# life-ufes/multimodal-model-skin-lesion-classifier

Hardware: AMD Instinct MI355X
Metric: images/sec fwd+bwd, ResNet-50+crossattention bs=256 (higher is better)
Workload: dtype bf16; 1 GPU; ResNet-50 + one-hot(20) + crossattention, 224x224, train step incl. Adam; per_gpu_batch=256, global_batch=256, parallelism=dp1, weights=random init (torchvision / timm / transformers layouts), unfreeze_weights=unfrozen_weights, linear_dtype=fp32

## Files before the change

### include/mmskin.h

```cpp
#ifndef MMSKIN_H
#define MMSKIN_H
#include <stdint.h>

#ifdef __cplusplus
extern "C" {
#endif

#define MMSKIN_F32 0
#define MMSKIN_BF16 1

const char* mmskin_last_error(void);
int mmskin_version(void);

typedef struct mmskin_backbone* mmskin_backbone_t;
int mmskin_backbone_create(const char* arch, int batch, int height, int width, int dtype, mmskin_backbone_t* out);
void mmskin_backbone_destroy(mmskin_backbone_t h);
int mmskin_backbone_num_tensors(mmskin_backbone_t h, int kind );
int mmskin_backbone_tensor_info(mmskin_backbone_t h, int kind, int index, char* name, int name_cap,
                                int64_t* offset, int64_t* numel, int* ndim, int64_t* shape4);
int64_t mmskin_backbone_param_numel(mmskin_backbone_t h);
int64_t mmskin_backbone_buffer_numel(mmskin_backbone_t h);
int64_t mmskin_backbone_workspace_bytes(mmskin_backbone_t h);
int mmskin_backbone_feature_dim(mmskin_backbone_t h);
int mmskin_backbone_feature_hw(mmskin_backbone_t h, int* out_h, int* out_w);
// ... 112 lines not shown
                                  void* stream);
int64_t mmskin_adaptive_avgpool_workspace_bytes(int N, int C, int H, int W);
int mmskin_adaptive_avgpool_forward(const float* x, float* out, int N, int C, int H, int W, int dtype, void* workspace, void* stream);
int mmskin_adaptive_avgpool_backward(const float* dout, float* dx, int N, int C, int H, int W, int dtype, void* workspace, void* stream);
int64_t mmskin_stem_workspace_bytes(int N, int H, int W);
int mmskin_stem_forward(const float* x, const float* w, const float* gamma, const float* beta, float* y, int N, int H,
                        int W, float eps, int dtype, void* workspace, void* stream);
int mmskin_stem_backward(const float* dy, const float* x, const float* w, const float* gamma, const float* beta,
                         float* dw, float* dgamma, float* dbeta, int N, int H, int W, float eps, int dtype,
                         void* workspace, void* stream);

int mmskin_linear_forward(const float* x, const float* w, const float* b, float* y, int M, int K, int N, int relu,
                          void* stream);
int mmskin_linear_backward(const float* dy, const float* x, const float* w, const float* y_relu, float* dy_scratch,
                           float* dx, float* dw, float* db, int M, int K, int N, void* stream);
int mmskin_linear_gelu_backward(const float* dh, const float* x, const float* w, const float* z, float* dy_scratch, float* dx, float* dw,
                                float* db, int M, int K, int N, void* stream);
int mmskin_linear_x16_pitch(int M, int K, int N);
enum { MMSKIN_LINEAR_SMALL = 0, MMSKIN_LINEAR_BIG_F32 = 1, MMSKIN_LINEAR_BIG_BF16 = 2, MMSKIN_LINEAR_PADDED_BF16 = 3 };
int mmskin_linear_route(int M, int K, int N);
int mmskin_linear_forward_keep(const float* x, const float* w, const float* b, const float* res, float* y, void* x16_keep, int M, int K,
                               int N, int relu, void* stream);
int mmskin_linear_backward_keep(const float* dy, const void* x16, const float* w, const float* y_relu, const float* z_gelu, float* dy_scratch,
                                float* dx, float* dw, float* db, int M, int K, int N, void* stream);
int mmskin_gelu_forward_bf16(const float* z, void* h16, int64_t rows, int cols, int cols_pad, void* stream);
int mmskin_linear_forward_x16(const void* x16, const float* w, const float* b, const float* res, float* y, int M, int K, int N, int relu,
                              void* stream);
int mmskin_star_relu_forward_bf16(const float* z, const float* s, const float* b, void* h16, int64_t rows, int cols, int cols_pad,
                                  void* stream);
int mmskin_linear_star_relu_backward_keep(const float* dh, const void* x16, const float* w, const float* z, const float* s, float* dsb,
// ... 201 lines not shown
```

### multimodal-model-skin-lesion-classifier_amd/csrc/linear.hip

```cpp
#include <stdlib.h>
#include <string.h>

#include "../../include/mmskin.h"
#include "conv.h"
#include "head_internal.h"

float* head_scratch(size_t bytes, int slot) {
  constexpr int MAXDEV = 16;
  static float* buf[2][MAXDEV] = {};
  static size_t cap[2][MAXDEV] = {};
  int d = 0;
  if (hipGetDevice(&d) != hipSuccess || d < 0 || d >= MAXDEV) return nullptr;
  if (bytes > cap[slot][d]) {
    if (buf[slot][d]) (void)hipFree(buf[slot][d]);
    size_t want = bytes < (size_t)(8 << 20) ? (size_t)(8 << 20) : bytes;
    if (hipMalloc((void**)&buf[slot][d], want) != hipSuccess) { buf[slot][d] = nullptr; cap[slot][d] = 0; return nullptr; }
    cap[slot][d] = want;
  }
  return buf[slot][d];
}
__global__ void split_reduce_kernel(const float* __restrict__ part, float* __restrict__ out, int S, int64_t n) {
  for (int64_t i = blockIdx.x * (int64_t)blockDim.x + threadIdx.x; i < n; i += (int64_t)gridDim.x * blockDim.x) {
    float t = 0.f;
    for (int s2 = 0; s2 < S; ++s2) t += part[(int64_t)s2 * n + i];
// ... 68 lines not shown
                                                       int64_t sbk, int64_t ldc, int relu, int kchunk, int64_t sab,
                                                       int64_t sbb, int64_t scb) {
  __shared__ float As[LG_LDS];
  __shared__ float Bs[LG_LDS];
  if (kchunk < 0) {
    a += (int64_t)blockIdx.z * sab; b += (int64_t)blockIdx.z * sbb; c += (int64_t)blockIdx.z * scb;
  }
  if (kchunk > 0) {
    const int kb = blockIdx.z * kchunk;
    a += (int64_t)kb * sak; b += (int64_t)kb * sbk;
    c += (int64_t)blockIdx.z * M * ldc;
    K = min(kchunk, K - kb);
  }
  gemm_f32_tile<A_KC, B_KC>(a, b, c, bias, M, N, K, sam, sak, sbn, sbk, ldc, relu, blockIdx.x, blockIdx.y, As, Bs);
}
__global__ __launch_bounds__(256) void linear_bwd_small_kernel(const float* __restrict__ g, const float* __restrict__ w, const float* __restrict__ x,
                                                               float* __restrict__ dx, float* __restrict__ dw, float* __restrict__ db, int M, int K,
                                                               int N, int nx_dx, int n_dx, int nx_dw, int n_dw) {
  __shared__ float As[LG_LDS];
  __shared__ float Bs[LG_LDS];
  int b = blockIdx.x;
  if (b < n_dx) {
    gemm_f32_tile<true, false>(g, w, dx, nullptr, M, K, N, N, 1, 1, K, K, 0, b % nx_dx, b / nx_dx, As, Bs);
    return;
  }
  b -= n_dx;
  if (b < n_dw) {
    gemm_f32_tile<false, false>(g, x, dw, nullptr, N, K, M, 1, N, 1, K, K, 0, b % nx_dw, b / nx_dw, As, Bs);
    return;
  }
  b -= n_dw;
  const int cx = threadIdx.x & 31, ry = threadIdx.x >> 5, n = b * 32 + cx;
  float s0 = 0.f, s1 = 0.f, s2 = 0.f, s3 = 0.f;
  if (n < N) {
    int m = ry;
    for (; m + 24 < M; m += 32) {
      s0 += g[(int64_t)m * N + n]; s1 += g[(int64_t)(m + 8) * N + n]; s2 += g[(int64_t)(m + 16) * N + n]; s3 += g[(int64_t)(m + 24) * N + n];
    }
    for (; m < M; m += 8) s0 += g[(int64_t)m * N + n];
  }
  As[ry * 32 + cx] = (s0 + s1) + (s2 + s3);
  __syncthreads();
  if (ry == 0 && n < N) {
    float t = 0.f;
#pragma unroll
    for (int i = 0; i < 8; ++i) t += As[i * 32 + cx];
    db[n] = t;
  }
}

static int gemm_f32(const float* a, const float* b, float* c, const float* bias, int M, int N, int K, int64_t sam,
                    int64_t sak, int64_t sbn, int64_t sbk, int64_t ldc, int relu, hipStream_t st, int batch = 1,
                    int64_t sab = 0, int64_t sbb = 0, int64_t scb = 0) {
  if (M <= 0 || N <= 0) return MMSKIN_OK;
  dim3 grid(ceil_div(N, LG_T), ceil_div(M, LG_T));
  const bool akc = sak == 1, bkc = sbk == 1;
  int S = 1, kchunk = 0;
  float* out = c;
  const int tiles = grid.x * grid.y;
  if (batch > 1) {
    grid.z = batch;
  } else if (K >= 4096 && tiles < 256 && !bias && !relu && ldc == N) {
    S = ceil_div(512, tiles);
// ... 480 lines not shown
  }
  if (path == LIN_BIG_F32) {
    ConvShape s = {M, 1, 1, K, N, 1, 1, 1, 0};
    FwdFuse f; f.bias = b; f.relu = relu == 1; f.gelu = relu == 2;
    return launch_conv_fwd<float>(s, x, w, y, nullptr, nullptr, st, (b || relu) ? &f : nullptr);
  }
  rc = gemm_f32(x, w, y, b, M, N, K, K, 1, K, 1, N, relu == 1, st);
  if (rc || relu != 2) return rc;
  return mmskin_gelu_forward(y, y, (int64_t)M * N, stream);
}

struct LinearBwdOpt {
  const void* x16_kept = nullptr;
  const float* star_s = nullptr;
  float* star_sb = nullptr;
};
static int linear_backward_impl(const float* dy, const float* x, const float* w, const float* y_relu, const float* z_gelu, float* dy_scratch,
                                float* dx, float* dw, float* db, int M, int K, int N, void* stream, const LinearBwdOpt& o = LinearBwdOpt()) {
  ARG_CHECK(dy && M > 0 && K > 0 && N > 0, "linear_backward: bad argument");
  ARG_CHECK(!(y_relu && z_gelu), "linear_backward: one activation");
  hipStream_t st = ST(stream);
  const float* g = dy;
  const LinearPath path = linear_path(M, K, N);
  const bool bf16_gemm = linear_bf16_gemm(path);
  ARG_CHECK(!o.x16_kept || bf16_gemm, "linear_backward: the kept bf16 operand belongs to the bf16 large-GEMM path (mode changed since the forward?)");
  ARG_CHECK(!o.star_s || (bf16_gemm && z_gelu && o.star_sb), "linear_backward: StarReLU needs the bf16 large-GEMM path, z and the scalar gradients");
  int rc;
  if (z_gelu && !bf16_gemm) {
    ARG_CHECK(dy_scratch, "linear_backward: dy_scratch required with z_gelu");
    if ((rc = mmskin_gelu_backward(dy, z_gelu, dy_scratch, (int64_t)M * N, stream))) return rc;
    g = dy_scratch; z_gelu = nullptr;
  }
  if (y_relu) {
    ARG_CHECK(dy_scratch, "linear_backward: dy_scratch required with y_relu");
    hipLaunchKernelGGL(relu_mask_kernel, dim3(grid1d((int64_t)M * N)), dim3(256), 0, st, dy, y_relu, dy_scratch, (int64_t)M * N);
    HIP_CHECK_RET(hipGetLastError());
    g = dy_scratch;
  }
  if (bf16_gemm) {
    const bool padded = path == LIN_PADDED_BF16;
    const int Kp = padded ? pad64(K) : K, Np = padded ? pad64(N) : N;
    ConvShape s = {M, 1, 1, Kp, Np, 1, 1, 1, 0};
    const size_t slab_bytes = conv_wgrad_slab_bytes(s);
    const size_t star_floats = o.star_s ? (size_t)2 * colsum4_blocks(M, Np / 4) : 0;
    bf16_t *g16 = nullptr, *t16 = nullptr, *w16 = nullptr;
    WgradSlab slab = {nullptr, slab_bytes / sizeof(float)};
    float *star_part = nullptr, *part = nullptr;
    const bool placed = carve_scratch([&](Carver& c) {
      g16 = c.take<bf16_t>((size_t)M * Np);
      t16 = c.take<bf16_t>((size_t)M * Kp);
      w16 = c.take<bf16_t>((size_t)Np * Kp);
      slab.p = reinterpret_cast<float*>(c.take<unsigned char>(slab_bytes));
      if (star_floats) star_part = c.take<float>(star_floats);
// ... 40 lines not shown
    });
    if (!placed) { mmskin_set_error("linear_backward: scratch allocation failed"); return MMSKIN_ERR_HIP; }
    if (dx) {
      ARG_CHECK(w, "linear_backward: w required for dx");
      hipLaunchKernelGGL(transpose_f32_kernel, dim3(ceil_div(K, 32), ceil_div(N, 32)), dim3(32, 8), 0, st, w, wt, N, K);
      HIP_CHECK_RET(hipGetLastError());
      if ((rc = launch_conv_dgrad<float>(s, g, wt, dx, (const float*)nullptr, st))) return rc;
    }
    if (dw) {
      ARG_CHECK(x, "linear_backward: x required for dw");
      if ((rc = launch_conv_wgrad<float>(s, g, x, slab, dw, st))) return rc;
    }
    if (db && (rc = colsum(g, db, M, N, st))) return rc;
    return MMSKIN_OK;
  }
  if (M < 4096 && (dx || dw || db)) {
    ARG_CHECK((!dx || w) && (!dw || x), "linear_backward: w / x required");
    const int nx_dx = ceil_div(K, LG_T), n_dx = dx ? nx_dx * ceil_div(M, LG_T) : 0;
    const int nx_dw = ceil_div(K, LG_T), n_dw = dw ? nx_dw * ceil_div(N, LG_T) : 0;
    const int n_db = db ? ceil_div(N, 32) : 0;
    hipLaunchKernelGGL(linear_bwd_small_kernel, dim3(n_dx + n_dw + n_db), dim3(256), 0, st, g, w, x, dx, dw, db, M, K, N, nx_dx, n_dx, nx_dw, n_dw);
    HIP_CHECK_RET(hipGetLastError());
    return MMSKIN_OK;
  }
  if (dx) {
    ARG_CHECK(w, "linear_backward: w required for dx");
    if ((rc = gemm_f32(g, w, dx, nullptr, M, K, N, N, 1, 1, K, K, 0, st))) return rc;
  }
  if (dw) {
    ARG_CHECK(x, "linear_backward: x required for dw");
    if ((rc = gemm_f32(g, x, dw, nullptr, N, K, M, 1, N, 1, K, K, 0, st))) return rc;
  }
  if (db && (rc = colsum(g, db, M, N, st))) return rc;
  return MMSKIN_OK;
}

// ... 71 lines not shown
            "linear_lane: dtype / activation");
  ARG_CHECK(drop_p >= 0.f && drop_p < 1.f, "linear_lane: dropout probability %f", (double)drop_p);
  ARG_CHECK(linear_path(M, K, N) == LIN_BIG_BF16, "linear_lane: M=%d K=%d N=%d is off the large bf16 GEMM path (rows >= 2048, 64-multiple widths, "
            "MMSKIN_LINEAR_DTYPE=bf16)", M, K, N);
  const bool tr = gamma || residual || drop_p > 0.f;
  ARG_CHECK(!tr || (y_dtype == 0 && N % 128 == 0), "linear_lane: residual / layer scale / dropout need an fp32 result and N %% 128 == 0");
  FwdFuse f; f.bias = b; f.relu = act == 1; f.gelu = act == 2;
  f.gamma = gamma; f.res_f32 = residual; f.drop_p = drop_p; f.seed = seed; f.offset = offset;
  return linear_big_bf16_ex(x, x_dtype, w, w_dtype, f, b || act || tr, y, y_dtype, M, K, N, "linear_lane", ST(stream));
}

int mmskin_linear_backward(const float* dy, const float* x, const float* w, const float* y_relu, float* dy_scratch,
                           float* dx, float* dw, float* db, int M, int K, int N, void* stream) {
  return linear_backward_impl(dy, x, w, y_relu, nullptr, dy_scratch, dx, dw, db, M, K, N, stream);
}
int mmskin_linear_gelu_backward(const float* dh, const float* x, const float* w, const float* z, float* dy_scratch, float* dx, float* dw,
                                float* db, int M, int K, int N, void* stream) {
  ARG_CHECK(z, "linear_gelu_backward: z required");
  return linear_backward_impl(dh, x, w, nullptr, z, dy_scratch, dx, dw, db, M, K, N, stream);
}
int mmskin_linear_backward_keep(const float* dy, const void* x16, const float* w, const float* y_relu, const float* z_gelu, float* dy_scratch,
                                float* dx, float* dw, float* db, int M, int K, int N, void* stream) {
  ARG_CHECK(x16, "linear_backward_keep: x16 required");
  LinearBwdOpt o; o.x16_kept = x16;
  return linear_backward_impl(dy, nullptr, w, y_relu, z_gelu, dy_scratch, dx, dw, db, M, K, N, stream, o);
}

int mmskin_linear_star_relu_backward_keep(const float* dh, const void* x16, const float* w, const float* z, const float* s, float* dsb,
                                          float* dx, float* dw, float* db, int M, int K, int N, void* stream) {
  ARG_CHECK(x16 && z && s && dsb, "linear_star_relu_backward_keep: x16, z, s and dsb required");
// ... 25 lines not shown
```

### multimodal-model-skin-lesion-classifier_amd/mmskin/_lib.py

```python
import ctypes
import os
import re

_HERE = os.path.dirname(os.path.abspath(__file__))
LIB_PATH = os.path.join(os.path.dirname(_HERE), "libmmskin_hip.so")
HEADER_PATH = os.path.join(os.path.dirname(os.path.dirname(_HERE)), "include", "mmskin.h")

F32, BF16 = 0, 1
LINEAR_SMALL, LINEAR_BIG_F32, LINEAR_BIG_BF16, LINEAR_PADDED_BF16 = 0, 1, 2, 3
WG_STAGED, WG_TAPS3, WG_RING, WG_RING3 = 0, 1, 2, 3
WGR_DIRECT, WGR_LANES = 0, 1
CG_TILE128, CG_BIG256, CG_PIPE, CG_C64, CG_STEM7 = 0, 1, 2, 3, 4

_lib = None

c_f = ctypes.c_void_p
_i, _i64, _f = ctypes.c_int, ctypes.c_int64, ctypes.c_float
_u64 = ctypes.c_uint64
_P = ctypes.c_void_p

_SIGNATURES = {
    "mmskin_last_error": (ctypes.c_char_p, []),
    "mmskin_version": (_i, []),
    "mmskin_backbone_create": (_i, [ctypes.c_char_p, _i, _i, _i, _i, ctypes.POINTER(_P)]),
    "mmskin_backbone_destroy": (None, [_P]),
    "mmskin_backbone_num_tensors": (_i, [_P, _i]),
    "mmskin_backbone_tensor_info": (_i, [_P, _i, _i, ctypes.c_char_p, _i, ctypes.POINTER(_i64),
                                         ctypes.POINTER(_i64), ctypes.POINTER(_i), ctypes.POINTER(_i64)]),
    "mmskin_backbone_param_numel": (_i64, [_P]),
    "mmskin_backbone_buffer_numel": (_i64, [_P]),
    "mmskin_backbone_workspace_bytes": (_i64, [_P]),
    "mmskin_backbone_feature_dim": (_i, [_P]),
    "mmskin_backbone_feature_hw": (_i, [_P, _P, _P]),
    "mmskin_backbone_set_option": (_i, [_P, ctypes.c_char_p, _i]),
# ... 60 lines not shown
    "mmskin_slice_stats_workspace_bytes": (_i64, [_i64, _i, _i, _i]),
    "mmskin_col_reduce_scratch_doubles": (_i64, [_i64]),
    "mmskin_col_reduce_scratch_check": (_i, [_i, _i, _i, _i64]),
    "mmskin_slice_stats": (_i, [_P, _i64, _i, _i, _i, _P, _P, _i, _P, _P]),
    "mmskin_maxpool2_relu_workspace_bytes": (_i64, [_i] * 4),
    "mmskin_maxpool2_relu_forward": (_i, [_P] * 3 + [_i] * 5 + [_P, _P]),
    "mmskin_maxpool2_relu_backward": (_i, [_P] * 3 + [_i] * 5 + [_P, _P]),
    "mmskin_adaptive_avgpool_workspace_bytes": (_i64, [_i] * 4),
    "mmskin_adaptive_avgpool_forward": (_i, [_P] * 2 + [_i] * 5 + [_P, _P]),
    "mmskin_adaptive_avgpool_backward": (_i, [_P] * 2 + [_i] * 5 + [_P, _P]),
    "mmskin_stem_workspace_bytes": (_i64, [_i] * 3),
    "mmskin_stem_forward": (_i, [_P] * 5 + [_i] * 3 + [_f, _i, _P, _P]),
    "mmskin_stem_backward": (_i, [_P] * 8 + [_i] * 3 + [_f, _i, _P, _P]),
    "mmskin_linear_forward": (_i, [_P] * 4 + [_i] * 4 + [_P]),
    "mmskin_linear_backward": (_i, [_P] * 8 + [_i] * 3 + [_P]),
    "mmskin_linear_gelu_backward": (_i, [_P] * 8 + [_i] * 3 + [_P]),
    "mmskin_linear_x16_pitch": (_i, [_i, _i, _i]),
    "mmskin_linear_route": (_i, [_i, _i, _i]),
    "mmskin_linear_forward_keep": (_i, [_P] * 6 + [_i] * 4 + [_P]),
    "mmskin_linear_backward_keep": (_i, [_P] * 9 + [_i] * 3 + [_P]),
    "mmskin_gelu_forward_bf16": (_i, [_P, _P, _i64, _i, _i, _P]),
    "mmskin_linear_forward_x16": (_i, [_P] * 5 + [_i] * 4 + [_P]),
    "mmskin_layernorm_forward": (_i, [_P] * 6 + [_i, _i, _f, _i, _P]),
    "mmskin_layernorm_backward": (_i, [_P] * 9 + [_i, _i, _i, _P]),
    "mmskin_sigmoid_gate_forward": (_i, [_P] * 3 + [_i64, _P]),
    "mmskin_sigmoid_gate_backward": (_i, [_P] * 5 + [_i64, _P]),
    "mmskin_gated_mix_forward": (_i, [_P] * 4 + [_i64, _P]),
    "mmskin_gated_mix_backward": (_i, [_P] * 7 + [_i64, _P]),
    "mmskin_metablock_gate_forward": (_i, [_P] * 4 + [_i64, _P]),
    "mmskin_metablock_gate_backward": (_i, [_P] * 7 + [_i64, _P]),
# ... 138 lines not shown
```

### multimodal-model-skin-lesion-classifier_amd/mmskin/nn.py

```python
import torch
import torch.nn as nn

from . import ops


class HipLinear(nn.Linear):
    def __init__(self, in_features, out_features, bias=True, fuse_relu=False):
        super().__init__(in_features, out_features, bias=bias)
        self.fuse_relu = fuse_relu

    def forward(self, x):
        return ops.linear(x, self.weight, self.bias, self.fuse_relu)

    def extra_repr(self):
        return super().extra_repr() + (", fused_relu=True" if self.fuse_relu else "")


class HipLayerNorm(nn.LayerNorm):
    def __init__(self, normalized_shape, fuse_relu=False):
        super().__init__(normalized_shape)
        self.fuse_relu = fuse_relu

    def forward(self, x):
        return ops.layernorm(x, self.weight, self.bias, self.eps, self.fuse_relu)
# ... 45 lines not shown
            v = ops.linear_rows(value.reshape(B, D), W, Bv, 2 * D, 3 * D)
            o = ops.linear(v, self.out_proj.weight, self.out_proj.bias).reshape(1, B, D)
            if Lq != 1:
                o = o.expand(Lq, B, D)
        else:
            q = ops.linear(query.reshape(Lq * B, D), W[:D], Bv[:D] if Bv is not None else None)
            k = ops.linear(key.reshape(Lk * B, D), W[D:2 * D], Bv[D:2 * D] if Bv is not None else None)
            v = ops.linear(value.reshape(Lk * B, D), W[2 * D:], Bv[2 * D:] if Bv is not None else None)
            split = lambda t, L: t.reshape(L, B, H, D // H).permute(1, 2, 0, 3).contiguous()
            a = ops.attention(split(q, Lq), split(k, Lk), split(v, Lk), self.dropout, self.training)
            a = a.permute(2, 0, 1, 3).reshape(Lq * B, D)
            o = ops.linear(a, self.out_proj.weight, self.out_proj.bias).reshape(Lq, B, D)
        if self.batch_first:
            o = o.transpose(0, 1)
        return o, None
```

### multimodal-model-skin-lesion-classifier_amd/mmskin/ops.py

```python
import ctypes
import weakref

import numpy as np
import torch

from . import _lib
from ._autograd import (_dropout_counter, _dropout_state, _dtype_code, _f32c, _need_gpu, _needs_grad, get_linear_dtype,
                        no_second_order)
from ._lib import call, ptr, stream
from .attention import (LongAttentionFn, _bmm, attention, attention_blhd, attention_packed, attention_route,
                        channel_attention, channel_attention_ok, window_attention, window_attention_ok)


def set_linear_dtype(name):
    call("mmskin_set_linear_dtype", {"fp32": _lib.F32, "float32": _lib.F32, "bf16": _lib.BF16, "bfloat16": _lib.BF16}[name.lower()])


def _linear_forward(x, w, b, res, act, want_keep):
    x2 = _f32c(x).reshape(-1, x.shape[-1])
    w = _f32c(w)
    M, K = x2.shape
    N = w.shape[0]
    y = torch.empty((M, N), device=x.device, dtype=torch.float32)
    pitch = _lib.load().mmskin_linear_x16_pitch(M, K, N) if want_keep else 0
# ... 60 lines not shown
             M, K, N, 0, stream())
        ctx.save_for_backward(x2 if ctx.needs_input_grad[1] else None, w)
        ctx.rows, ctx.mk, ctx.xshape = (r0, r1), (M, K), x.shape
        ctx.bias = None if b is None else (b.shape, b.dtype)
        return y.reshape(*x.shape[:-1], N)

    @staticmethod
    def backward(ctx, dy):
        xs, w = ctx.saved_tensors
        (r0, r1), (M, K) = ctx.rows, ctx.mk
        N = r1 - r0
        dy2 = _f32c(dy).reshape(M, N)
        need_x, need_w = ctx.needs_input_grad[0], ctx.needs_input_grad[1]
        need_b = ctx.bias is not None and ctx.needs_input_grad[2]
        dx = torch.empty((M, K), device=dy.device, dtype=torch.float32) if need_x else None
        nw, nb = (w.numel() if need_w else 0), (ctx.bias[0].numel() if need_b else 0)
        flat = torch.zeros(nw + nb, device=dy.device, dtype=torch.float32) if nw + nb else None
        dw = flat[:nw].view_as(w) if need_w else None
        db = flat[nw:].view(ctx.bias[0]) if need_b else None
        call("mmskin_linear_backward", ptr(dy2), ptr(xs), w.data_ptr() + 4 * r0 * K, None, None, ptr(dx),
             (dw.data_ptr() + 4 * r0 * K) if need_w else None, (db.data_ptr() + 4 * r0) if need_b else None, M, K, N, stream())
        return (dx.reshape(ctx.xshape) if need_x else None), dw, db, None, None


def linear_rows(x, w, b, r0, r1):
    if x.dtype != torch.float32 or not x.is_cuda:
        return linear(x, w[r0:r1], b[r0:r1] if b is not None else None)
    return LinearRowsFn.apply(x, w, b, r0, r1)


def _rows_f32_or_bf16(x):
    x2 = x.reshape(-1, x.shape[-1]).contiguous()
    return x2 if x2.dtype in (torch.float32, torch.bfloat16) else x2.float()


def lane_dtype(x, module=None, *tensors):
    if not x.is_cuda or get_linear_dtype() != "bf16":
        return None
    params = tuple(module.parameters()) if module is not None else ()
    return None if _needs_grad(x, *params, *tensors) else torch.bfloat16


def _linear_ex(x, w, b, act, out_dtype):
# ... 944 lines not shown
```

### multimodal-model-skin-lesion-classifier_amd/models/gatedResidualBlock.py

```python
import os
import sys

import torch.nn as nn

_PKG = os.path.dirname(os.path.dirname(os.path.abspath(__file__)))
if _PKG not in sys.path:
    sys.path.insert(0, _PKG)

from mmskin import ops
from mmskin.nn import HipDropout, HipLayerNorm, HipLinear, HipMultiheadAttention


class GatedAlteredResidualBlock(nn.Module):
    def __init__(self, dim, dropout=0.1):
        super().__init__()
        self.norm = HipLayerNorm(dim)
        self.attn = HipMultiheadAttention(embed_dim=dim, num_heads=8, batch_first=False)
        self.dropout = HipDropout(dropout)
        self.gate_linear = HipLinear(dim, dim)

    def forward(self, q, k, v):
        a = self.dropout(self.attn(q, k, v)[0])
        z = self.gate_linear(q)
        return self.norm(ops.gated_mix(z, a.expand_as(q) if a.shape != q.shape else a, q))


class StackedGatedResidualBlock(nn.Module):
    def __init__(self, dim, depth=4, dropout=0.1):
        super().__init__()
        self.blocks = nn.ModuleList(
            [GatedAlteredResidualBlock(dim=dim, dropout=dropout) for _ in range(depth)])

    def forward(self, q, k=None, v=None):
        k = q if k is None else k
        v = q if v is None else v
        for block in self.blocks:
            q = block(q, k, v)
        return q
```

### multimodal-model-skin-lesion-classifier_amd/models/multimodalIntraInterModal.py

```python
import os
import sys

import torch
import torch.nn as nn

_HERE = os.path.dirname(os.path.abspath(__file__))
_PKG = os.path.dirname(_HERE)
for _p in (_PKG, _HERE):
    if _p not in sys.path:
        sys.path.insert(0, _p)

from gatedResidualBlock import GatedAlteredResidualBlock, StackedGatedResidualBlock
from loadImageModelClassifier import loadModels
from metablock import MetaBlock
from mmskin import ops
from mmskin.nn import FusedAway, HipDropout, HipLayerNorm, HipLinear, HipMultiheadAttention

_RG = "att-intramodal+residual+cross-attention-metadados"


class MultimodalModel(nn.Module):
    def __init__(self, num_classes, num_heads, device, cnn_model_name, text_model_name, batch_size=32,
                 common_dim=512, text_encoder_dim_output=512, vocab_size=91,
                 unfreeze_weights="frozen_weights", attention_mecanism="concatenation", n=2):
        super().__init__()
        self.device = device
        self.common_dim = common_dim
        self.num_heads = num_heads
        self.attention_mecanism = attention_mecanism
        self.n = n
        self.vocab_size = vocab_size
# ... 71 lines not shown
            img_feat = img_feat.mean(dim=(-2, -1))
        return img_feat

    def forward(self, image, text_metadata):
        return self.fuse(self.encode_image(image), text_metadata)

    def fuse(self, img_feat, text_metadata):
        mech = self.attention_mecanism
        needs_meta = mech not in ("no-metadata", "no-metadata-without-mlp")
        if mech == "no-metadata-without-mlp":
            return self.fc_visual_only(img_feat)
        txt_feat = self._metadata_features(text_metadata) if needs_meta else None
        if mech == "metablock":
            return self.fc_mlp_module_after_metablock_fusion_module(self.meta_block(img_feat, txt_feat))

        P_i = self.image_projector(img_feat).unsqueeze(0)
        if mech == "no-metadata":
            return self.fc_fusion(P_i.squeeze(0))
        P_t = self.text_projector(txt_feat).unsqueeze(0)

        isa, tsa = self.image_self_attention, self.text_self_attention
        ica, tca = self.image_cross_attention, self.text_cross_attention
        ires, tres = self.image_residual, self.text_residual
        att = lambda mod, q, kv: mod(q, kv, kv)[0]
        fuse = lambda a, b: self.fc_fusion(ops.concat2(a.squeeze(0), b.squeeze(0)))
        f2o = self.fc_fusion_proj_feat2output

        if mech == "concatenation":
            return fuse(P_i, P_t)
        if mech == "weighted":
            return fuse(ops.sigmoid_gate(self.img_gate(P_i), P_i), ops.sigmoid_gate(self.txt_gate(P_t), P_t))
        if mech == "rg-att2fusefeatures":
            return f2o(ires(P_t, P_i, P_i).squeeze(0))
        if mech == "rg-att":
            return fuse(ires(P_i, P_t, P_t), tres(P_t, P_i, P_i))
        if mech == "cross-attention-only":
            return fuse(att(ica, P_i, P_t), att(tca, P_t, P_i))
        if mech == "residual+cross-attention-metadados":
            R_i, R_t = ires(P_i, P_i, P_i), tres(P_t, P_t, P_t)
            return fuse(att(ica, R_i, R_t), att(tca, R_t, R_i))

        A_i, A_t = att(isa, P_i, P_i), att(tsa, P_t, P_t)
        if mech == "att-intramodal":
            return fuse(A_i, A_t)
        if mech == "att-intramodal+residual":
            return fuse(ires(P_i, A_i, A_i), tres(P_t, A_t, A_t))
        if mech in ("crossattention", "gfcam", "cross-weights-after-crossattention"):
            C_i, C_t = att(ica, A_i, A_t), att(tca, A_t, A_i)
            if mech == "crossattention":
                return fuse(C_i, C_t)
            z_i, z_t = self.img_gate(C_i), self.txt_gate(C_t)
            if mech == "gfcam":
                return fuse(ops.sigmoid_gate(z_i, C_i), ops.sigmoid_gate(z_t, C_t))
            return fuse(ops.sigmoid_gate(z_t, C_i), ops.sigmoid_gate(z_i, C_t))
        if mech.startswith(_RG):
            R_i, R_t = ires(P_i, A_i, A_i), tres(P_t, A_t, A_t)
            X_i, X_t = att(ica, R_i, R_t), att(tca, R_t, R_i)
            tail = mech[len(_RG):]
            if tail == "":
                return fuse(X_i, X_t)
            if tail == "+rg-att2fusefeatures":
                return f2o(ires(X_t, X_i, X_i).squeeze(0))
            if tail == "+metablock":
                return f2o(self.meta_block(X_i.squeeze(0), X_t.squeeze(0)))
            if tail == "+att-intramodal+residual":
                A2_i, A2_t = att(isa, X_i, X_i), att(tsa, X_t, X_t)
                return fuse(ires(X_i, A2_i, A2_i), tres(X_t, A2_t, A2_t))
        raise ValueError(f"Attention mechanism '{mech}' not implemented.")
```

Baseline: 14710 images/sec.

## Batch paired image/text head linears and attention into single paired kernel launches

Adds forward and backward paired-linear kernels that run two independent small fp32 linear problems (image and text branch) in one launch using a 2-D grid. The crossattention model's projectors, self/cross attention (sequence-length-1 shortcut through the value and out projections) and gates now go through these paired paths. Backward also folds the zeroing of unused weight-gradient rows into the same kernel instead of separate memsets. The aim is to cut kernel-launch and Python dispatch overhead in the tiny head layers, at the cost of more complex autograd plumbing and grids that idle when the two problems differ in size.

Measured after the change: 14840 images/sec (median of 6 runs). Within noise of the previous version (+0.9%).

```diff
diff --git a/include/mmskin.h b/include/mmskin.h
--- a/include/mmskin.h
+++ b/include/mmskin.h
@@ -150,6 +150,17 @@
                           void* stream);
 int mmskin_linear_backward(const float* dy, const float* x, const float* w, const float* y_relu, float* dy_scratch,
                            float* dx, float* dw, float* db, int M, int K, int N, void* stream);
+typedef struct mmskin_linear_fwd_desc {
+  const float* x; const float* w; const float* b; float* y;
+  int M, K, N, act, r0, r1;
+} mmskin_linear_fwd_desc;
+typedef struct mmskin_linear_bwd_desc {
+  const float* dy; const float* x; const float* w; const float* y_relu; float* dy_scratch; float* dx; float* dw; float* db;
+  int M, K, N, r0, r1;
+} mmskin_linear_bwd_desc;
+int mmskin_linear_forward_pair(const mmskin_linear_fwd_desc* a, const mmskin_linear_fwd_desc* b, void* stream);
+int mmskin_linear_backward_pair(const mmskin_linear_bwd_desc* a, const mmskin_linear_bwd_desc* b, void* stream);
+int64_t mmskin_linear_pair_launches(void);
 int mmskin_linear_gelu_backward(const float* dh, const float* x, const float* w, const float* z, float* dy_scratch, float* dx, float* dw,
                                 float* db, int M, int K, int N, void* stream);
 int mmskin_linear_x16_pitch(int M, int K, int N);
diff --git a/multimodal-model-skin-lesion-classifier_amd/csrc/linear.hip b/multimodal-model-skin-lesion-classifier_amd/csrc/linear.hip
--- a/multimodal-model-skin-lesion-classifier_amd/csrc/linear.hip
+++ b/multimodal-model-skin-lesion-classifier_amd/csrc/linear.hip
@@ -106,39 +106,83 @@
   }
   gemm_f32_tile<A_KC, B_KC>(a, b, c, bias, M, N, K, sam, sak, sbn, sbk, ldc, relu, blockIdx.x, blockIdx.y, As, Bs);
 }
-__global__ __launch_bounds__(256) void linear_bwd_small_kernel(const float* __restrict__ g, const float* __restrict__ w, const float* __restrict__ x,
-                                                               float* __restrict__ dx, float* __restrict__ dw, float* __restrict__ db, int M, int K,
-                                                               int N, int nx_dx, int n_dx, int nx_dw, int n_dw) {
+#define LB_ZERO 4096
+struct LinBwdProb {
+  const float *g, *w, *x;
+  float *dx, *dw, *db;
+  int M, K, N;
+  int nx_dx, n_dx, nx_dw, n_dw, n_db, n_zero;
+  int r0, nw;
+};
+static inline int lin_bwd_blocks(const LinBwdProb& p) { return p.n_dx + p.n_dw + p.n_db + p.n_zero; }
+__device__ __forceinline__ void linear_bwd_small_block(const LinBwdProb& p, int b, float* As, float* Bs) {
+  const float* __restrict__ g = p.g;
+  const int M = p.M, K = p.K, N = p.N;
+  if (b < p.n_dx) {
+    gemm_f32_tile<true, false>(g, p.w, p.dx, nullptr, M, K, N, N, 1, 1, K, K, 0, b % p.nx_dx, b / p.nx_dx, As, Bs);
+    return;
+  }
+  b -= p.n_dx;
+  if (b < p.n_dw) {
+    gemm_f32_tile<false, false>(g, p.x, p.dw, nullptr, N, K, M, 1, N, 1, K, K, 0, b % p.nx_dw, b / p.nx_dw, As, Bs);
+    return;
+  }
+  b -= p.n_dw;
+  if (b < p.n_db) {
+    const int cx = threadIdx.x & 31, ry = threadIdx.x >> 5, n = b * 32 + cx;
+    float s0 = 0.f, s1 = 0.f, s2 = 0.f, s3 = 0.f;
+    if (n < N) {
+      int m = ry;
+      for (; m + 24 < M; m += 32) {
+        s0 += g[(int64_t)m * N + n]; s1 += g[(int64_t)(m + 8) * N + n]; s2 += g[(int64_t)(m + 16) * N + n]; s3 += g[(int64_t)(m + 24) * N + n];
+      }
+      for (; m < M; m += 8) s0 += g[(int64_t)m * N + n];
+    }
+    As[ry * 32 + cx] = (s0 + s1) + (s2 + s3);
+    __syncthreads();
+    if (ry == 0 && n < N) {
+      float t = 0.f;
+#pragma unroll
+      for (int i = 0; i < 8; ++i) t += As[i * 32 + cx];
+      p.db[n] = t;
+    }
+    return;
+  }
+  b -= p.n_db;
+  const int64_t zw = p.dw ? (int64_t)(p.nw - N) * K : 0, zt = zw + (p.db ? p.nw - N : 0);
+  const int64_t lo = (int64_t)p.r0 * K;
+  float* __restrict__ dw0 = p.dw - lo;
+  float* __restrict__ db0 = p.db - p.r0;
+  const int64_t end = min((int64_t)(b + 1) * LB_ZERO, zt);
+  for (int64_t i = (int64_t)b * LB_ZERO + threadIdx.x; i < end; i += 256) {
+    if (i < zw) dw0[i < lo ? i : i + (int64_t)N * K] = 0.f;
+    else { const int64_t j = i - zw; db0[j < p.r0 ? j : j + N] = 0.f; }
+  }
+}
+__global__ __launch_bounds__(256) void linear_bwd_small_kernel(LinBwdProb p) {
   __shared__ float As[LG_LDS];
   __shared__ float Bs[LG_LDS];
-  int b = blockIdx.x;
-  if (b < n_dx) {
-    gemm_f32_tile<true, false>(g, w, dx, nullptr, M, K, N, N, 1, 1, K, K, 0, b % nx_dx, b / nx_dx, As, Bs);
-    return;
-  }
-  b -= n_dx;
-  if (b < n_dw) {
-    gemm_f32_tile<false, false>(g, x, dw, nullptr, N, K, M, 1, N, 1, K, K, 0, b % nx_dw, b / nx_dw, As, Bs);
-    return;
-  }
-  b -= n_dw;
-  const int cx = threadIdx.x & 31, ry = threadIdx.x >> 5, n = b * 32 + cx;
-  float s0 = 0.f, s1 = 0.f, s2 = 0.f, s3 = 0.f;
-  if (n < N) {
-    int m = ry;
-    for (; m + 24 < M; m += 32) {
-      s0 += g[(int64_t)m * N + n]; s1 += g[(int64_t)(m + 8) * N + n]; s2 += g[(int64_t)(m + 16) * N + n]; s3 += g[(int64_t)(m + 24) * N + n];
-    }
-    for (; m < M; m += 8) s0 += g[(int64_t)m * N + n];
-  }
-  As[ry * 32 + cx] = (s0 + s1) + (s2 + s3);
-  __syncthreads();
-  if (ry == 0 && n < N) {
-    float t = 0.f;
-#pragma unroll
-    for (int i = 0; i < 8; ++i) t += As[i * 32 + cx];
-    db[n] = t;
-  }
+  linear_bwd_small_block(p, blockIdx.x, As, Bs);
+}
+struct LinFwdProb {
+  const float *x, *w, *b;
+  float* y;
+  int M, K, N, relu, nx, nblk;
+};
+__global__ __launch_bounds__(256) void linear_fwd_pair_kernel(LinFwdProb p0, LinFwdProb p1) {
+  __shared__ float As[LG_LDS];
+  __shared__ float Bs[LG_LDS];
+  const LinFwdProb& p = blockIdx.y ? p1 : p0;
+  const int b = blockIdx.x;
+  if (b >= p.nblk) return;
+  gemm_f32_tile<true, true>(p.x, p.w, p.y, p.b, p.M, p.N, p.K, p.K, 1, p.K, 1, p.N, p.relu, b % p.nx, b / p.nx, As, Bs);
+}
+__global__ __launch_bounds__(256) void linear_bwd_pair_kernel(LinBwdProb p0, LinBwdProb p1) {
+  __shared__ float As[LG_LDS];
+  __shared__ float Bs[LG_LDS];
+  const LinBwdProb& p = blockIdx.y ? p1 : p0;
+  if ((int)blockIdx.x >= p.n_dx + p.n_dw + p.n_db + p.n_zero) return;
+  linear_bwd_small_block(p, blockIdx.x, As, Bs);
 }
 
 static int gemm_f32(const float* a, const float* b, float* c, const float* bias, int M, int N, int K, int64_t sam,
@@ -649,7 +693,34 @@
   const void* x16_kept = nullptr;
   const float* star_s = nullptr;
   float* star_sb = nullptr;
+  int r0 = 0, nw = 0;
 };
+static inline bool linear_bwd_one_launch(LinearPath path, int M) { return path == LIN_SMALL && M < 4096; }
+static inline bool linear_fwd_one_launch(LinearPath path, int K, int act) { return path == LIN_SMALL && K < 4096 && act != 2; }
+static LinBwdProb lin_bwd_prob(const float* g, const float* w, const float* x, float* dx, float* dw, float* db, int M, int K, int N, int r0,
+                               int nw) {
+  LinBwdProb p = {g, w, x, dx, dw, db, M, K, N};
+  p.nx_dx = ceil_div(K, LG_T); p.n_dx = dx ? p.nx_dx * ceil_div(M, LG_T) : 0;
+  p.nx_dw = ceil_div(K, LG_T); p.n_dw = dw ? p.nx_dw * ceil_div(N, LG_T) : 0;
+  p.n_db = db ? ceil_div(N, 32) : 0;
+  const int64_t zeros = nw > N ? (dw ? (int64_t)(nw - N) * K : 0) + (db ? nw - N : 0) : 0;
+  p.n_zero = (int)((zeros + LB_ZERO - 1) / LB_ZERO);
+  p.r0 = r0; p.nw = nw;
+  return p;
+}
+static int relu_mask(const float* dy, const float* y, float* out, int64_t n, hipStream_t st) {
+  hipLaunchKernelGGL(relu_mask_kernel, dim3(grid1d(n)), dim3(256), 0, st, dy, y, out, n);
+  HIP_CHECK_RET(hipGetLastError());
+  return MMSKIN_OK;
+}
+static int zero_outside_rows(float* dw, float* db, int K, int N, int r0, int nw, hipStream_t st) {
+  const size_t head = (size_t)r0, tail = (size_t)(nw - r0 - N);
+  if (dw && head) HIP_CHECK_RET(hipMemsetAsync(dw - head * K, 0, head * K * sizeof(float), st));
+  if (dw && tail) HIP_CHECK_RET(hipMemsetAsync(dw + (size_t)N * K, 0, tail * K * sizeof(float), st));
+  if (db && head) HIP_CHECK_RET(hipMemsetAsync(db - head, 0, head * sizeof(float), st));
+  if (db && tail) HIP_CHECK_RET(hipMemsetAsync(db + N, 0, tail * sizeof(float), st));
+  return MMSKIN_OK;
+}
 static int linear_backward_impl(const float* dy, const float* x, const float* w, const float* y_relu, const float* z_gelu, float* dy_scratch,
                                 float* dx, float* dw, float* db, int M, int K, int N, void* stream, const LinearBwdOpt& o = LinearBwdOpt()) {
   ARG_CHECK(dy && M > 0 && K > 0 && N > 0, "linear_backward: bad argument");
@@ -668,10 +739,10 @@
   }
   if (y_relu) {
     ARG_CHECK(dy_scratch, "linear_backward: dy_scratch required with y_relu");
-    hipLaunchKernelGGL(relu_mask_kernel, dim3(grid1d((int64_t)M * N)), dim3(256), 0, st, dy, y_relu, dy_scratch, (int64_t)M * N);
-    HIP_CHECK_RET(hipGetLastError());
+    if ((rc = relu_mask(dy, y_relu, dy_scratch, (int64_t)M * N, st))) return rc;
     g = dy_scratch;
   }
+  if (o.nw > N && !linear_bwd_one_launch(path, M) && (rc = zero_outside_rows(dw, db, K, N, o.r0, o.nw, st))) return rc;
   if (bf16_gemm) {
     const bool padded = path == LIN_PADDED_BF16;
     const int Kp = padded ? pad64(K) : K, Np = padded ? pad64(N) : N;
@@ -742,12 +813,10 @@
     if (db && (rc = colsum(g, db, M, N, st))) return rc;
     return MMSKIN_OK;
   }
-  if (M < 4096 && (dx || dw || db)) {
+  if (linear_bwd_one_launch(path, M) && (dx || dw || db)) {
     ARG_CHECK((!dx || w) && (!dw || x), "linear_backward: w / x required");
-    const int nx_dx = ceil_div(K, LG_T), n_dx = dx ? nx_dx * ceil_div(M, LG_T) : 0;
-    const int nx_dw = ceil_div(K, LG_T), n_dw = dw ? nx_dw * ceil_div(N, LG_T) : 0;
-    const int n_db = db ? ceil_div(N, 32) : 0;
-    hipLaunchKernelGGL(linear_bwd_small_kernel, dim3(n_dx + n_dw + n_db), dim3(256), 0, st, g, w, x, dx, dw, db, M, K, N, nx_dx, n_dx, nx_dw, n_dw);
+    const LinBwdProb p = lin_bwd_prob(g, w, x, dx, dw, db, M, K, N, o.r0, o.nw);
+    hipLaunchKernelGGL(linear_bwd_small_kernel, dim3(lin_bwd_blocks(p)), dim3(256), 0, st, p);
     HIP_CHECK_RET(hipGetLastError());
     return MMSKIN_OK;
   }
@@ -849,6 +918,76 @@
                            float* dx, float* dw, float* db, int M, int K, int N, void* stream) {
   return linear_backward_impl(dy, x, w, y_relu, nullptr, dy_scratch, dx, dw, db, M, K, N, stream);
 }
+static int64_t g_pair_launches = 0;
+int64_t mmskin_linear_pair_launches(void) { return g_pair_launches; }
+static bool fwd_desc_ok(const mmskin_linear_fwd_desc* d) {
+  return d && d->x && d->w && d->y && d->M > 0 && d->K > 0 && d->r0 >= 0 && d->r0 < d->r1 && d->r1 <= d->N && d->act >= 0 && d->act <= 2;
+}
+static int linear_forward_desc(const mmskin_linear_fwd_desc& d, void* stream) {
+  LinOperands op; op.x = d.x; op.w = d.w + (size_t)d.r0 * d.K;
+  return linear_forward_impl(op, d.b ? d.b + d.r0 : nullptr, nullptr, d.y, d.M, d.K, d.r1 - d.r0, d.act, stream);
+}
+int mmskin_linear_forward_pair(const mmskin_linear_fwd_desc* a, const mmskin_linear_fwd_desc* b, void* stream) {
+  ARG_CHECK(fwd_desc_ok(a) && fwd_desc_ok(b), "linear_forward_pair: bad descriptor");
+  const mmskin_linear_fwd_desc* d[2] = {a, b};
+  bool pair = true;
+  for (int i = 0; i < 2; ++i) pair = pair && linear_fwd_one_launch(linear_path(d[i]->M, d[i]->K, d[i]->r1 - d[i]->r0), d[i]->K, d[i]->act);
+  if (!pair) {
+    const int rc = linear_forward_desc(*a, stream);
+    return rc ? rc : linear_forward_desc(*b, stream);
+  }
+  LinFwdProb p[2];
+  for (int i = 0; i < 2; ++i) {
+    const int N = d[i]->r1 - d[i]->r0, K = d[i]->K;
+    p[i] = {d[i]->x, d[i]->w + (size_t)d[i]->r0 * K, d[i]->b ? d[i]->b + d[i]->r0 : nullptr, d[i]->y, d[i]->M, K, N, d[i]->act == 1,
+            ceil_div(N, LG_T), ceil_div(N, LG_T) * ceil_div(d[i]->M, LG_T)};
+  }
+  hipLaunchKernelGGL(linear_fwd_pair_kernel, dim3(p[0].nblk > p[1].nblk ? p[0].nblk : p[1].nblk, 2), dim3(256), 0, ST(stream), p[0], p[1]);
+  HIP_CHECK_RET(hipGetLastError());
+  ++g_pair_launches;
+  return MMSKIN_OK;
+}
+static bool bwd_desc_ok(const mmskin_linear_bwd_desc* d) {
+  return d && d->dy && d->M > 0 && d->K > 0 && d->r0 >= 0 && d->r0 < d->r1 && d->r1 <= d->N && (!d->dx || d->w) && (!d->dw || d->x) &&
+         (!d->y_relu || d->dy_scratch);
+}
+static int linear_backward_desc(const mmskin_linear_bwd_desc& d, void* stream) {
+  const size_t r0 = (size_t)d.r0;
+  LinearBwdOpt o; o.r0 = d.r0; o.nw = d.N;
+  return linear_backward_impl(d.dy, d.x, d.w ? d.w + r0 * d.K : nullptr, d.y_relu, nullptr, d.dy_scratch, d.dx, d.dw ? d.dw + r0 * d.K : nullptr,
+                              d.db ? d.db + r0 : nullptr, d.M, d.K, d.r1 - d.r0, stream, o);
+}
+int mmskin_linear_backward_pair(const mmskin_linear_bwd_desc* a, const mmskin_linear_bwd_desc* b, void* stream) {
+  ARG_CHECK(bwd_desc_ok(a) && (!b || bwd_desc_ok(b)), "linear_backward_pair: bad descriptor");
+  if (!b) return linear_backward_desc(*a, stream);
+  const mmskin_linear_bwd_desc* d[2] = {a, b};
+  bool pair = true;
+  for (int i = 0; i < 2; ++i)
+    pair = pair && linear_bwd_one_launch(linear_path(d[i]->M, d[i]->K, d[i]->r1 - d[i]->r0), d[i]->M) && (d[i]->dx || d[i]->dw || d[i]->db);
+  if (!pair) {
+    const int rc = linear_backward_desc(*a, stream);
+    return rc ? rc : linear_backward_desc(*b, stream);
+  }
+  hipStream_t st = ST(stream);
+  LinBwdProb p[2];
+  for (int i = 0; i < 2; ++i) {
+    const int N = d[i]->r1 - d[i]->r0, K = d[i]->K, M = d[i]->M;
+    const size_t r0 = (size_t)d[i]->r0;
+    const float* g = d[i]->dy;
+    if (d[i]->y_relu) {
+      const int rc = relu_mask(g, d[i]->y_relu, d[i]->dy_scratch, (int64_t)M * N, st);
+      if (rc) return rc;
+      g = d[i]->dy_scratch;
+    }
+    p[i] = lin_bwd_prob(g, d[i]->w ? d[i]->w + r0 * K : nullptr, d[i]->x, d[i]->dx, d[i]->dw ? d[i]->dw + r0 * K : nullptr,
+                        d[i]->db ? d[i]->db + r0 : nullptr, M, K, N, d[i]->r0, d[i]->N);
+  }
+  const int n0 = lin_bwd_blocks(p[0]), n1 = lin_bwd_blocks(p[1]);
+  hipLaunchKernelGGL(linear_bwd_pair_kernel, dim3(n0 > n1 ? n0 : n1, 2), dim3(256), 0, st, p[0], p[1]);
+  HIP_CHECK_RET(hipGetLastError());
+  ++g_pair_launches;
+  return MMSKIN_OK;
+}
 int mmskin_linear_gelu_backward(const float* dh, const float* x, const float* w, const float* z, float* dy_scratch, float* dx, float* dw,
                                 float* db, int M, int K, int N, void* stream) {
   ARG_CHECK(z, "linear_gelu_backward: z required");
diff --git a/multimodal-model-skin-lesion-classifier_amd/mmskin/_lib.py b/multimodal-model-skin-lesion-classifier_amd/mmskin/_lib.py
--- a/multimodal-model-skin-lesion-classifier_amd/mmskin/_lib.py
+++ b/multimodal-model-skin-lesion-classifier_amd/mmskin/_lib.py
@@ -18,6 +18,15 @@
 _i, _i64, _f = ctypes.c_int, ctypes.c_int64, ctypes.c_float
 _u64 = ctypes.c_uint64
 _P = ctypes.c_void_p
+
+
+class LinearFwdDesc(ctypes.Structure):
+    _fields_ = [(n, _P) for n in ("x", "w", "b", "y")] + [(n, _i) for n in ("M", "K", "N", "act", "r0", "r1")]
+
+
+class LinearBwdDesc(ctypes.Structure):
+    _fields_ = [(n, _P) for n in ("dy", "x", "w", "y_relu", "dy_scratch", "dx", "dw", "db")] + [(n, _i) for n in ("M", "K", "N", "r0", "r1")]
+
 
 _SIGNATURES = {
     "mmskin_last_error": (ctypes.c_char_p, []),
@@ -108,6 +117,9 @@
     "mmskin_stem_backward": (_i, [_P] * 8 + [_i] * 3 + [_f, _i, _P, _P]),
     "mmskin_linear_forward": (_i, [_P] * 4 + [_i] * 4 + [_P]),
     "mmskin_linear_backward": (_i, [_P] * 8 + [_i] * 3 + [_P]),
+    "mmskin_linear_forward_pair": (_i, [ctypes.POINTER(LinearFwdDesc), ctypes.POINTER(LinearFwdDesc), _P]),
+    "mmskin_linear_backward_pair": (_i, [ctypes.POINTER(LinearBwdDesc), ctypes.POINTER(LinearBwdDesc), _P]),
+    "mmskin_linear_pair_launches": (_i64, []),
     "mmskin_linear_gelu_backward": (_i, [_P] * 8 + [_i] * 3 + [_P]),
     "mmskin_linear_x16_pitch": (_i, [_i, _i, _i]),
     "mmskin_linear_route": (_i, [_i, _i, _i]),
diff --git a/multimodal-model-skin-lesion-classifier_amd/mmskin/nn.py b/multimodal-model-skin-lesion-classifier_amd/mmskin/nn.py
--- a/multimodal-model-skin-lesion-classifier_amd/mmskin/nn.py
+++ b/multimodal-model-skin-lesion-classifier_amd/mmskin/nn.py
@@ -83,3 +83,27 @@
         if self.batch_first:
             o = o.transpose(0, 1)
         return o, None
+
+
+def hooked(*mods):
+    g = torch.nn.modules.module
+    if g._global_forward_hooks or g._global_forward_pre_hooks or g._global_backward_hooks or g._global_backward_pre_hooks:
+        return True
+    return any(m._forward_hooks or m._forward_pre_hooks or m._backward_hooks or m._backward_pre_hooks for m in mods)
+
+
+def linear_pair(mod_a, x_a, mod_b, x_b):
+    if hooked(mod_a, mod_b):
+        return mod_a(x_a), mod_b(x_b)
+    return ops.paired_linear((x_a, mod_a.weight, mod_a.bias), (x_b, mod_b.weight, mod_b.bias), relu=(mod_a.fuse_relu, mod_b.fuse_relu))
+
+
+def attention_pair(mod_a, q_a, kv_a, mod_b, q_b, kv_b):
+    if mod_a.batch_first or mod_b.batch_first or kv_a.shape[0] != 1 or kv_b.shape[0] != 1 or hooked(mod_a, mod_b):
+        return mod_a(q_a, kv_a, kv_a)[0], mod_b(q_b, kv_b, kv_b)[0]
+    Da, Db = mod_a.embed_dim, mod_b.embed_dim
+    v_a, v_b = ops.paired_linear((kv_a.reshape(-1, Da), mod_a.in_proj_weight, mod_a.in_proj_bias, 2 * Da, 3 * Da),
+                                 (kv_b.reshape(-1, Db), mod_b.in_proj_weight, mod_b.in_proj_bias, 2 * Db, 3 * Db))
+    o_a, o_b = ops.paired_linear((v_a, mod_a.out_proj.weight, mod_a.out_proj.bias), (v_b, mod_b.out_proj.weight, mod_b.out_proj.bias))
+    shape = lambda o, q, D: o.reshape(1, -1, D) if q.shape[0] == 1 else o.reshape(1, -1, D).expand(q.shape[0], -1, D)
+    return shape(o_a, q_a, Da), shape(o_b, q_b, Db)
diff --git a/multimodal-model-skin-lesion-classifier_amd/mmskin/ops.py b/multimodal-model-skin-lesion-classifier_amd/mmskin/ops.py
--- a/multimodal-model-skin-lesion-classifier_amd/mmskin/ops.py
+++ b/multimodal-model-skin-lesion-classifier_amd/mmskin/ops.py
@@ -98,12 +98,10 @@
         need_x, need_w = ctx.needs_input_grad[0], ctx.needs_input_grad[1]
         need_b = ctx.bias is not None and ctx.needs_input_grad[2]
         dx = torch.empty((M, K), device=dy.device, dtype=torch.float32) if need_x else None
-        nw, nb = (w.numel() if need_w else 0), (ctx.bias[0].numel() if need_b else 0)
-        flat = torch.zeros(nw + nb, device=dy.device, dtype=torch.float32) if nw + nb else None
-        dw = flat[:nw].view_as(w) if need_w else None
-        db = flat[nw:].view(ctx.bias[0]) if need_b else None
-        call("mmskin_linear_backward", ptr(dy2), ptr(xs), w.data_ptr() + 4 * r0 * K, None, None, ptr(dx),
-             (dw.data_ptr() + 4 * r0 * K) if need_w else None, (db.data_ptr() + 4 * r0) if need_b else None, M, K, N, stream())
+        dw = torch.empty_like(w) if need_w else None
+        db = torch.empty(ctx.bias[0], device=dy.device, dtype=torch.float32) if need_b else None
+        d = _lib.LinearBwdDesc(_dp(dy2), _dp(xs), _dp(w), None, None, _dp(dx), _dp(dw), _dp(db), M, K, w.shape[0], r0, r1)
+        call("mmskin_linear_backward_pair", ctypes.byref(d), None, stream())
         return (dx.reshape(ctx.xshape) if need_x else None), dw, db, None, None
 
 
@@ -111,6 +109,71 @@
     if x.dtype != torch.float32 or not x.is_cuda:
         return linear(x, w[r0:r1], b[r0:r1] if b is not None else None)
     return LinearRowsFn.apply(x, w, b, r0, r1)
+
+
+def _dp(t):
+    return None if t is None else t.data_ptr()
+
+
+@no_second_order
+class PairedLinearFn(torch.autograd.Function):
+
+    @staticmethod
+    def forward(ctx, xa, wa, ba, rows_a, relu_a, xb, wb, bb, rows_b, relu_b):
+        descs, ys, saved, ctx.meta = [], [], [], []
+        for i, (x, w, b, rows, relu) in enumerate(((xa, wa, ba, rows_a, relu_a), (xb, wb, bb, rows_b, relu_b))):
+            _need_gpu(x, "paired_linear")
+            x2 = _f32c(x).reshape(-1, x.shape[-1])
+            w = _f32c(w)
+            b = _f32c(b) if b is not None else None
+            r0, r1 = rows if rows is not None else (0, w.shape[0])
+            M, K = x2.shape
+            y = torch.empty((M, r1 - r0), device=x.device, dtype=torch.float32)
+            descs.append(_lib.LinearFwdDesc(_dp(x2), _dp(w), _dp(b), _dp(y), M, K, w.shape[0], int(bool(relu)), r0, r1))
+            ys.append(y.reshape(*x.shape[:-1], r1 - r0))
+            saved += [x2 if ctx.needs_input_grad[5 * i + 1] else None, w, y if relu else None]
+            ctx.meta.append((r0, r1, M, K, x.shape, b is not None))
+        call("mmskin_linear_forward_pair", ctypes.byref(descs[0]), ctypes.byref(descs[1]), stream())
+        ctx.save_for_backward(*saved)
+        ctx.set_materialize_grads(False)
+        return ys[0], ys[1]
+
+    @staticmethod
+    def backward(ctx, *dys):
+        saved, need = ctx.saved_tensors, ctx.needs_input_grad
+        descs, keep, grads = [], [], []
+        for i, dy in enumerate(dys):
+            xs, w, y = saved[3 * i:3 * i + 3]
+            r0, r1, M, K, xshape, has_bias = ctx.meta[i]
+            need_x, need_w, need_b = need[5 * i], need[5 * i + 1], has_bias and need[5 * i + 2]
+            if dy is None or not (need_x or need_w or need_b):
+                grads += [None] * 5
+                continue
+            dy2 = _f32c(dy).reshape(M, r1 - r0)
+            dx = torch.empty((M, K), device=dy.device, dtype=torch.float32) if need_x else None
+            dw = torch.empty_like(w) if need_w else None
+            db = torch.empty(w.shape[0], device=dy.device, dtype=torch.float32) if need_b else None
+            scratch = torch.empty_like(dy2) if y is not None else None
+            descs.append(_lib.LinearBwdDesc(_dp(dy2), _dp(xs), _dp(w), _dp(y), _dp(scratch), _dp(dx), _dp(dw), _dp(db), M, K, w.shape[0], r0, r1))
+            keep.append((dy2, scratch))
+            grads += [dx.reshape(xshape) if need_x else None, dw, db, None, None]
+        if descs:
+            call("mmskin_linear_backward_pair", ctypes.byref(descs[0]), ctypes.byref(descs[1]) if len(descs) == 2 else None, stream())
+        return tuple(grads)
+
+
+def paired_linear(a, b, relu=(False, False)):
+    one = lambda s, r: linear_rows(*s) if len(s) == 5 else linear(s[0], s[1], s[2], r)
+    for s, r in zip((a, b), relu):
+        if s[1].numel() != s[1].shape[0] * s[0].shape[-1]:
+            raise _lib.MMSkinError(f"linear: input of width {s[0].shape[-1]} for a weight of shape {tuple(s[1].shape)}")
+        if len(s) == 5 and r:
+            raise _lib.MMSkinError("paired_linear: the row-block form has no fused ReLU")
+    fp32 = all(s[0].is_cuda and s[0].dtype == torch.float32 for s in (a, b)) and get_linear_dtype() == "fp32"
+    if not fp32 or _needs_grad(*a[:3]) != _needs_grad(*b[:3]):
+        return one(a, relu[0]), one(b, relu[1])
+    return PairedLinearFn.apply(a[0], a[1], a[2], tuple(a[3:5]) if len(a) == 5 else None, relu[0],
+                                b[0], b[1], b[2], tuple(b[3:5]) if len(b) == 5 else None, relu[1])
 
 
 def _rows_f32_or_bf16(x):
diff --git a/multimodal-model-skin-lesion-classifier_amd/models/gatedResidualBlock.py b/multimodal-model-skin-lesion-classifier_amd/models/gatedResidualBlock.py
--- a/multimodal-model-skin-lesion-classifier_amd/models/gatedResidualBlock.py
+++ b/multimodal-model-skin-lesion-classifier_amd/models/gatedResidualBlock.py
@@ -8,7 +8,7 @@
     sys.path.insert(0, _PKG)
 
 from mmskin import ops
-from mmskin.nn import HipDropout, HipLayerNorm, HipLinear, HipMultiheadAttention
+from mmskin.nn import HipDropout, HipLayerNorm, HipLinear, HipMultiheadAttention, attention_pair, hooked, linear_pair
 
 
 class GatedAlteredResidualBlock(nn.Module):
@@ -22,7 +22,19 @@
     def forward(self, q, k, v):
         a = self.dropout(self.attn(q, k, v)[0])
         z = self.gate_linear(q)
+        return self._mix(z, a, q)
+
+    def _mix(self, z, a, q):
         return self.norm(ops.gated_mix(z, a.expand_as(q) if a.shape != q.shape else a, q))
+
+
+def gated_residual_pair(blk_a, q_a, kv_a, blk_b, q_b, kv_b):
+    if hooked(blk_a, blk_b):
+        return blk_a(q_a, kv_a, kv_a), blk_b(q_b, kv_b, kv_b)
+    a_a, a_b = attention_pair(blk_a.attn, q_a, kv_a, blk_b.attn, q_b, kv_b)
+    a_a, a_b = blk_a.dropout(a_a), blk_b.dropout(a_b)
+    z_a, z_b = linear_pair(blk_a.gate_linear, q_a, blk_b.gate_linear, q_b)
+    return blk_a._mix(z_a, a_a, q_a), blk_b._mix(z_b, a_b, q_b)
 
 
 class StackedGatedResidualBlock(nn.Module):
diff --git a/multimodal-model-skin-lesion-classifier_amd/models/multimodalIntraInterModal.py b/multimodal-model-skin-lesion-classifier_amd/models/multimodalIntraInterModal.py
--- a/multimodal-model-skin-lesion-classifier_amd/models/multimodalIntraInterModal.py
+++ b/multimodal-model-skin-lesion-classifier_amd/models/multimodalIntraInterModal.py
@@ -10,11 +10,11 @@
     if _p not in sys.path:
         sys.path.insert(0, _p)
 
-from gatedResidualBlock import GatedAlteredResidualBlock, StackedGatedResidualBlock
+from gatedResidualBlock import GatedAlteredResidualBlock, StackedGatedResidualBlock, gated_residual_pair
 from loadImageModelClassifier import loadModels
 from metablock import MetaBlock
 from mmskin import ops
-from mmskin.nn import FusedAway, HipDropout, HipLayerNorm, HipLinear, HipMultiheadAttention
+from mmskin.nn import FusedAway, HipDropout, HipLayerNorm, HipLinear, HipMultiheadAttention, attention_pair, linear_pair
 
 _RG = "att-intramodal+residual+cross-attention-metadados"
 
@@ -116,48 +116,48 @@
         if mech == "metablock":
             return self.fc_mlp_module_after_metablock_fusion_module(self.meta_block(img_feat, txt_feat))
 
-        P_i = self.image_projector(img_feat).unsqueeze(0)
         if mech == "no-metadata":
-            return self.fc_fusion(P_i.squeeze(0))
-        P_t = self.text_projector(txt_feat).unsqueeze(0)
+            return self.fc_fusion(self.image_projector(img_feat))
+        P_i, P_t = (p.unsqueeze(0) for p in linear_pair(self.image_projector, img_feat, self.text_projector, txt_feat))
 
         isa, tsa = self.image_self_attention, self.text_self_attention
         ica, tca = self.image_cross_attention, self.text_cross_attention
         ires, tres = self.image_residual, self.text_residual
-        att = lambda mod, q, kv: mod(q, kv, kv)[0]
+        att2, res2 = attention_pair, gated_residual_pair
         fuse = lambda a, b: self.fc_fusion(ops.concat2(a.squeeze(0), b.squeeze(0)))
         f2o = self.fc_fusion_proj_feat2output
 
         if mech == "concatenation":
             return fuse(P_i, P_t)
         if mech == "weighted":
-            return fuse(ops.sigmoid_gate(self.img_gate(P_i), P_i), ops.sigmoid_gate(self.txt_gate(P_t), P_t))
+            z_i, z_t = linear_pair(self.img_gate, P_i, self.txt_gate, P_t)
+            return fuse(ops.sigmoid_gate(z_i, P_i), ops.sigmoid_gate(z_t, P_t))
         if mech == "rg-att2fusefeatures":
             return f2o(ires(P_t, P_i, P_i).squeeze(0))
         if mech == "rg-att":
-            return fuse(ires(P_i, P_t, P_t), tres(P_t, P_i, P_i))
+            return fuse(*res2(ires, P_i, P_t, tres, P_t, P_i))
         if mech == "cross-attention-only":
-            return fuse(att(ica, P_i, P_t), att(tca, P_t, P_i))
+            return fuse(*att2(ica, P_i, P_t, tca, P_t, P_i))
         if mech == "residual+cross-attention-metadados":
-            R_i, R_t = ires(P_i, P_i, P_i), tres(P_t, P_t, P_t)
-            return fuse(att(ica, R_i, R_t), att(tca, R_t, R_i))
+            R_i, R_t = res2(ires, P_i, P_i, tres, P_t, P_t)
+            return fuse(*att2(ica, R_i, R_t, tca, R_t, R_i))
 
-        A_i, A_t = att(isa, P_i, P_i), att(tsa, P_t, P_t)
+        A_i, A_t = att2(isa, P_i, P_i, tsa, P_t, P_t)
         if mech == "att-intramodal":
             return fuse(A_i, A_t)
         if mech == "att-intramodal+residual":
-            return fuse(ires(P_i, A_i, A_i), tres(P_t, A_t, A_t))
+            return fuse(*res2(ires, P_i, A_i, tres, P_t, A_t))
         if mech in ("crossattention", "gfcam", "cross-weights-after-crossattention"):
-            C_i, C_t = att(ica, A_i, A_t), att(tca, A_t, A_i)
+            C_i, C_t = att2(ica, A_i, A_t, tca, A_t, A_i)
             if mech == "crossattention":
                 return fuse(C_i, C_t)
-            z_i, z_t = self.img_gate(C_i), self.txt_gate(C_t)
+            z_i, z_t = linear_pair(self.img_gate, C_i, self.txt_gate, C_t)
             if mech == "gfcam":
                 return fuse(ops.sigmoid_gate(z_i, C_i), ops.sigmoid_gate(z_t, C_t))
             return fuse(ops.sigmoid_gate(z_t, C_i), ops.sigmoid_gate(z_i, C_t))
         if mech.startswith(_RG):
-            R_i, R_t = ires(P_i, A_i, A_i), tres(P_t, A_t, A_t)
-            X_i, X_t = att(ica, R_i, R_t), att(tca, R_t, R_i)
+            R_i, R_t = res2(ires, P_i, A_i, tres, P_t, A_t)
+            X_i, X_t = att2(ica, R_i, R_t, tca, R_t, R_i)
             tail = mech[len(_RG):]
             if tail == "":
                 return fuse(X_i, X_t)
@@ -166,6 +166,6 @@
             if tail == "+metablock":
                 return f2o(self.meta_block(X_i.squeeze(0), X_t.squeeze(0)))
             if tail == "+att-intramodal+residual":
-                A2_i, A2_t = att(isa, X_i, X_i), att(tsa, X_t, X_t)
-                return fuse(ires(X_i, A2_i, A2_i), tres(X_t, A2_t, A2_t))
+                A2_i, A2_t = att2(isa, X_i, X_i, tsa, X_t, X_t)
+                return fuse(*res2(ires, X_i, A2_i, tres, X_t, A2_t))
         raise ValueError(f"Attention mechanism '{mech}' not implemented.")
```
